# SamsungLabs/SummaryMixing

Hardware: AMD Instinct MI355X
Metric: encoder frames/s (whole node), LibriSpeech Conformer-SummaryMixing (higher is better)
Workload: dtype bf16; 1 GPU; LibriSpeech Conformer-SummaryMixing C2b (12L, d_model=256, d_ffn=1024, SummaryMixing-fast, Swish) training step (fwd+bwd+grad-clip+AdamW); per_gpu_batch=128, enc_frames_per_utt=500, global_batch=128, valid_frames_rank0=49222, input=(B,T,640) N(0,1), wav_len U(0.5,1), zero padded, parallelism=dp1, init=xavier_normal seed 3407, residual_stream=float32 (torch autocast semantics, the reference's `precision: bf16`), launch=eager

## Files before the change

include/smx.h:

```cpp
#ifndef SMX_H_
#define SMX_H_

#include <stddef.h>
#include <stdint.h>

#ifdef __cplusplus
extern "C" {
#endif

#define SMX_VERSION 100

enum { SMX_OK = 0, SMX_EINVAL = -1, SMX_EUNSUPPORTED = -2, SMX_ELAUNCH = -3 };
enum { SMX_F32 = 0, SMX_BF16 = 1 };
enum { SMX_ACT_NONE = 0, SMX_ACT_GELU = 1, SMX_ACT_SWISH = 2, SMX_ACT_LEAKY_RELU = 3, SMX_ACT_RELU = 4 };
enum { SMX_C0_NONE = 0, SMX_C0_ROW = 1, SMX_C0_GROUP = 2, SMX_C0_MOD = 3 };
enum { SMX_GEMM_NT = 0,
       SMX_GEMM_NN = 1,
       SMX_GEMM_TN = 2   };
enum { SMX_OUT_T = 0, SMX_OUT_F32 = 1, SMX_OUT_ATOMIC_F32 = 2 };
enum { SMX_PAD_ZERO = 0, SMX_PAD_REFLECT = 1 };

int smx_version(void);
const char* smx_last_error(void);

// ... 157 lines not shown
  const void* R;       int64_t ldr;
  void* dX;            int64_t lddx;
  float* dgamma;       float* dbeta;
  void* workspace;
  void* dX2;           int64_t lddx2;
  const uint8_t* row_mask2;
  float alpha2;        float drop_p2;
  uint64_t drop_seed2;
  const uint64_t* epoch;
  const void* Z;       int64_t ldz;
  int32_t zact;        int32_t N;
  int32_t D;           int32_t pad_;
} smx_ln_bwd;
int smx_layernorm_bwd(const smx_ln_bwd* a, void* stream);
int smx_layernorm_bwd_blocks(int N);
size_t smx_layernorm_bwd_workspace(int N, int D);

int smx_dwconv1d_glu_fwd(int dtype, const void* P, int64_t ldp, const float* w, const float* bias,
                         const void* gate, int64_t ldg, void* Y, int64_t ldy, int B, int T, int D, int k, int glu,
                         int pad_mode, int chunk, void* stream);
int smx_dwconv1d_glu_fwd_drop(int dtype, const void* P, int64_t ldp, const float* w, const float* bias,
                              const void* gate, int64_t ldg, void* Y, int64_t ldy, int B, int T, int D, int k, int glu,
                              int pad_mode, int chunk, float drop_p, uint64_t drop_seed, const uint64_t* epoch, void* stream);
size_t smx_dwconv1d_glu_bwd_workspace(int B, int T, int D, int k);
int smx_dwconv1d_glu_bwd_partial_rows(int dtype, int B, int T, int D, int k, int glu, int pad_mode, int chunk, int has_gate);
int smx_dwconv1d_glu_bwd(int dtype, const void* dY, int64_t lddy, const void* P, int64_t ldp, const float* w,
                         const float* bias, const void* gate, int64_t ldg, void* dP, int64_t lddp, void* dgate,
                         int64_t lddg, float* dw, float* dbias, int B, int T, int D, int k, int glu, int pad_mode,
                         int chunk, void* workspace, void* stream);

int smx_dft_frames(const float* wav_padded, int64_t ldw, const float* basis_cos, const float* basis_sin, float* spec, int64_t lds,
                   int im_off, int B, int T, int n_fft, int hop, int rows_basis, void* stream);
int smx_frame_window(const float* wav, int64_t ldw, const float* window, float* frames, int B, int L, int T, int n_fft,
                     int hop, void* stream);
size_t smx_fbank_workspace(int B, int T, int n_mels);
int smx_mel_db(int out_dtype, const float* spec, int64_t lds, int im_off, const float* fb, int n_bins, int n_mels,
               float amin, float top_db, void* out, int B, int T, void* workspace, void* stream);
int smx_im2col_s2(int dtype, const void* x, void* col, int B, int T, int F, int C, int Kp, void* stream);
int smx_col2im_s2(int dtype, const void* dcol, void* dx, int B, int T, int F, int C, int Kp, void* stream);
size_t smx_conv1_ln_workspace(int B, int T, int F, int O);
int smx_conv1_ln_fwd(int dtype, const void* X, const float* W9, const float* bias, const float* gamma, const float* beta, float eps,
                     int act, void* Y, float* stats, int B, int T, int F, int O, void* stream);
int smx_conv1_ln_bwd(int dtype, const void* dA, const void* X, const float* W9, const float* bias, const float* gamma,
                     const float* beta, const float* stats, int act, float* grads, void* workspace, int B, int T, int F, int O,
                     void* stream);
int smx_linear_k16_fwd(int dtype, const void* X, const void* W, const float* bias, void* Y, int64_t N, int M, void* stream);
// ... 114 lines not shown
```

summarymixing_amd/_lib.py:

```python
import ctypes
import os

_HERE = os.path.dirname(os.path.abspath(__file__))
LIB_PATH = os.environ.get("SMX_LIB") or os.path.join(_HERE, "libsmx.so")

c_i, c_i64, c_f, c_vp, c_sz = ctypes.c_int, ctypes.c_int64, ctypes.c_float, ctypes.c_void_p, ctypes.c_size_t

F32, BF16 = 0, 1
ACT_NONE, ACT_GELU, ACT_SWISH, ACT_LEAKY_RELU, ACT_RELU = 0, 1, 2, 3, 4
C0_NONE, C0_ROW, C0_GROUP, C0_MOD = 0, 1, 2, 3
GEMM_NT, GEMM_NN, GEMM_TN = 0, 1, 2
OUT_T, OUT_F32, OUT_ATOMIC_F32 = 0, 1, 2
EPI_C0_POST = 1
EPI_ACT_GRAD = 2
EPI_LN_BWD = 4
EPI_LN_FWD = 8
IO_RES_F32, IO_LNX_F32, IO_LNFY_F32 = 1, 2, 4
PAD_ZERO, PAD_REFLECT = 0, 1
ACTS = {"none": ACT_NONE, "identity": ACT_NONE, "gelu": ACT_GELU, "swish": ACT_SWISH,
        "leaky_relu": ACT_LEAKY_RELU, "relu": ACT_RELU}


class ReduceJob(ctypes.Structure):
    _fields_ = [("src", c_vp), ("dst", c_vp), ("src_stride", c_i64), ("ldd", c_i64), ("nsrc", ctypes.c_int32),
# ... 92 lines not shown
    "smx_act_mask_bwd_workspace": (c_sz, [c_i, c_i]),
    "smx_act_mask_bwd": (c_i, [c_i, c_vp, c_i64, c_vp, c_i64, c_vp, c_vp, c_i64, c_i, c_i, c_i, c_f, c_vp, c_vp,
                               c_i64, c_i, c_f, ctypes.c_uint64, c_vp, c_vp, c_vp]),
    "smx_masked_mean_workspace": (c_sz, [c_i, c_i, c_i]),
    "smx_masked_mean_fwd": (c_i, [c_i, c_vp, c_i64, c_vp, c_vp, c_vp, c_i, c_i, c_i, c_i, c_vp, c_vp]),
    "smx_masked_mean_bwd": (c_i, [c_i, c_vp, c_vp, c_vp, c_i64, c_i, c_i, c_i, c_f, ctypes.c_uint64, c_vp, c_vp]),
    "smx_pool_bcast_ok": (c_i, [c_i, c_i, c_i]),
    "smx_pool_bcast": (c_i, [c_i, c_vp, c_i64, c_vp, c_vp, c_vp, c_vp, c_vp, c_i64, c_i, c_i, c_i, c_i, c_f, ctypes.c_uint64, c_vp, c_vp, c_i64,
                             c_vp, c_i, c_vp]),
    "smx_masked_mean_bwd_act": (c_i, [c_i, c_vp, c_vp, c_vp, c_i64, c_vp, c_i64, c_vp, c_i, c_i, c_i, c_i, c_vp]),
    "smx_chunk_mean_workspace": (c_sz, [c_i, c_i, c_i, c_i]),
    "smx_chunk_mean_fwd": (c_i, [c_i, c_vp, c_i64, c_vp, c_i64, c_i, c_i, c_i, c_i, c_i, c_vp, c_vp]),
    "smx_chunk_mean_bwd": (c_i, [c_i, c_vp, c_i64, c_vp, c_i64, c_i, c_i, c_i, c_i, c_i, c_vp, c_vp]),
    "smx_expdecay_mean_workspace": (c_sz, [c_i, c_i, c_i]),
    "smx_expdecay_mean_fwd": (c_i, [c_i, c_vp, c_i64, c_vp, c_i64, c_i, c_i, c_i, c_f, c_vp, c_vp]),
    "smx_expdecay_mean_bwd": (c_i, [c_i, c_vp, c_i64, c_vp, c_i64, c_i, c_i, c_i, c_f, c_vp, c_vp]),
    "smx_layernorm_fwd": (c_i, [ctypes.POINTER(LnFwd), c_vp]),
    "smx_layernorm_bwd_workspace": (c_sz, [c_i, c_i]),
    "smx_layernorm_bwd": (c_i, [ctypes.POINTER(LnBwd), c_vp]),
    "smx_dwconv1d_glu_fwd": (c_i, [c_i, c_vp, c_i64, c_vp, c_vp, c_vp, c_i64, c_vp, c_i64, c_i, c_i, c_i, c_i, c_i,
                                   c_i, c_i, c_vp]),
    "smx_dwconv1d_glu_fwd_drop": (c_i, [c_i, c_vp, c_i64, c_vp, c_vp, c_vp, c_i64, c_vp, c_i64, c_i, c_i, c_i, c_i, c_i,
                                        c_i, c_i, c_f, ctypes.c_uint64, c_vp, c_vp]),
    "smx_dwconv1d_glu_bwd_workspace": (c_sz, [c_i, c_i, c_i, c_i]),
    "smx_dwconv1d_glu_bwd_partial_rows": (c_i, [c_i] * 9),
    "smx_dwconv1d_glu_bwd": (c_i, [c_i, c_vp, c_i64, c_vp, c_i64, c_vp, c_vp, c_vp, c_i64, c_vp, c_i64, c_vp, c_i64,
                                   c_vp, c_vp, c_i, c_i, c_i, c_i, c_i, c_i, c_i, c_vp, c_vp]),
    "smx_dft_frames": (c_i, [c_vp, c_i64, c_vp, c_vp, c_vp, c_i64, c_i, c_i, c_i, c_i, c_i, c_i, c_vp]),
    "smx_frame_window": (c_i, [c_vp, c_i64, c_vp, c_vp, c_i, c_i, c_i, c_i, c_i, c_vp]),
    "smx_fbank_workspace": (c_sz, [c_i, c_i, c_i]),
    "smx_mel_db": (c_i, [c_i, c_vp, c_i64, c_i, c_vp, c_i, c_i, c_f, c_f, c_vp, c_i, c_i, c_vp, c_vp]),
    "smx_im2col_s2": (c_i, [c_i, c_vp, c_vp, c_i, c_i, c_i, c_i, c_i, c_vp]),
    "smx_col2im_s2": (c_i, [c_i, c_vp, c_vp, c_i, c_i, c_i, c_i, c_i, c_vp]),
    "smx_conv1_ln_workspace": (c_sz, [c_i, c_i, c_i, c_i]),
    "smx_conv1_ln_fwd": (c_i, [c_i, c_vp, c_vp, c_vp, c_vp, c_vp, c_f, c_i, c_vp, c_vp, c_i, c_i, c_i, c_i, c_vp]),
    "smx_conv1_ln_bwd": (c_i, [c_i, c_vp, c_vp, c_vp, c_vp, c_vp, c_vp, c_vp, c_i, c_vp, c_vp, c_i, c_i, c_i, c_i, c_vp]),
    "smx_linear_k16_fwd": (c_i, [c_i, c_vp, c_vp, c_vp, c_vp, c_i64, c_i, c_vp]),
    "smx_conv2d_s2_fwd": (c_i, [c_i, c_vp, c_vp, c_vp, c_vp, c_i, c_i, c_i, c_i, c_i, c_i, c_vp]),
    "smx_conv2d_s2_wgrad_workspace": (c_sz, [c_i, c_i, c_i, c_i, c_i]),
    "smx_conv2d_s2_wgrad": (c_i, [c_i, c_vp, c_vp, c_vp, c_vp, c_i, c_i, c_i, c_i, c_i, c_i, c_vp, c_vp]),
    "smx_conv2d_s2_dgrad": (c_i, [c_i, c_vp, c_vp, c_vp, c_i, c_i, c_i, c_i, c_i, c_i, c_vp]),
    "smx_axpby": (c_i, [c_i, c_f, c_vp, c_i64, c_f, c_vp, c_i64, c_vp, c_i64, c_i, c_i, c_vp]),
    "smx_dropout": (c_i, [c_i, c_vp, c_i64, c_vp, c_i64, c_i, c_i, c_f, ctypes.c_uint64, c_vp, c_vp]),
    "smx_add_rowtable": (c_i, [c_i, c_vp, c_i64, c_vp, c_i, c_i, c_i, c_vp]),
    "smx_cast_from_f32": (c_i, [c_i, c_vp, c_vp, c_i64, c_vp]),
    "smx_cast_to_f32": (c_i, [c_i, c_vp, c_vp, c_i64, c_vp]),
# ... 95 lines not shown
```

summarymixing_amd/csrc/dwconv.hip:

```cpp
#include "smx_common.h"

namespace smx {

constexpr int DW_TT = 64;
constexpr int DW_CT = 64;
constexpr int DW_KMAX = 33;
constexpr int DW_ROWS = DW_TT + DW_KMAX - 1;

struct DwParams {
  const void* P; long ldp;
  const float* w; const float* bias;
  const void* gate; long ldg;
  void* Y; long ldy;
  void* dP; long lddp;
  void* dgate; long lddg;
  float* dw; float* dbias;
  int B, T, D, k, glu, pad_mode, chunk;
  unsigned dthresh; float dscale; uint64_t dseed; const uint64_t* epoch;
};

__device__ __forceinline__ int map_frame(int tau, int T, int pad_mode) {
  if (tau >= 0 && tau < T) return tau;
  if (pad_mode == SMX_PAD_REFLECT) {
    int r = tau < 0 ? -tau : 2 * (T - 1) - tau;
    return (r >= 0 && r < T) ? r : -1;
  }
  return -1;
}

template <typename T>
__device__ __forceinline__ void fill_u(float (*u)[DW_CT], const DwParams& p, int b, int t0, int pad, int ch, int cl, int wv) {
  const T* P = reinterpret_cast<const T*>(p.P);
  const int rows = DW_TT + 2 * pad;
  for (int i = wv; i < rows; i += 4) {
    int src = map_frame(t0 - pad + i, p.T, p.pad_mode);
    float val = 0.f;
    if (src >= 0 && ch < p.D) {
      const T* row = P + ((long)b * p.T + src) * p.ldp;
      float a = to_f32(row[ch]);
      val = p.glu ? a * sigmoidf_(to_f32(row[p.D + ch])) : a;
    }
// ... 542 lines not shown
    if (drop_p > 0.f && rk != 2) return fail(SMX_EUNSUPPORTED, "smx_dwconv1d_glu_fwd_drop: fused output dropout needs the rolling CSGU kernel");
    if (rk == 2) {
      p.dthresh = (unsigned)((double)drop_p * 4294967296.0); p.dscale = 1.f / (1.f - drop_p); p.dseed = drop_seed; p.epoch = epoch;
      hipLaunchKernelGGL(dwconv_rollc_fwd, g1, dim3(256), 0, s, p, seg, nseg, gy);
    }
    else if (dtype == SMX_BF16) {
      if (chunk > 0) hipLaunchKernelGGL((dwconv_rolls_fwd<true>), g1, dim3(256), 0, s, p, seg, nseg, gy);
      else hipLaunchKernelGGL((dwconv_rolls_fwd<false>), g1, dim3(256), 0, s, p, seg, nseg, gy);
    } else if (chunk > 0) hipLaunchKernelGGL((dwconv_roll_fwd<float, true>), g1, dim3(256), 0, s, p, seg, nseg, gy);
    else hipLaunchKernelGGL((dwconv_roll_fwd<float, false>), g1, dim3(256), 0, s, p, seg, nseg, gy);
  } else if (drop_p > 0.f) {
    return fail(SMX_EUNSUPPORTED, "smx_dwconv1d_glu_fwd_drop: fused output dropout needs the rolling CSGU kernel");
  } else if (fast) {
    if (gate) {
      if (dtype == SMX_BF16) hipLaunchKernelGGL((dwconv_fwd_fast<bf16_t, 31, true>), grid, dim3(256), 0, s, p);
      else hipLaunchKernelGGL((dwconv_fwd_fast<float, 31, true>), grid, dim3(256), 0, s, p);
    } else {
      if (dtype == SMX_BF16) hipLaunchKernelGGL((dwconv_fwd_fast<bf16_t, 31, false>), grid, dim3(256), 0, s, p);
      else hipLaunchKernelGGL((dwconv_fwd_fast<float, 31, false>), grid, dim3(256), 0, s, p);
    }
  } else if (dtype == SMX_BF16) hipLaunchKernelGGL((dwconv_fwd_kernel<bf16_t>), grid, dim3(256), 0, s, p);
  else hipLaunchKernelGGL((dwconv_fwd_kernel<float>), grid, dim3(256), 0, s, p);
  return check_launch("smx_dwconv1d_glu_fwd");
}

static long tiled_rows(int B, int T, int D) {
  const int tiles_t = (T + DW_TT - 1) / DW_TT, ctiles = (D + DW_CT - 1) / DW_CT;
  long total = (long)B * tiles_t, gy = (1024 + ctiles - 1) / ctiles;
  if (gy > total) gy = total;
  if (gy < 1) gy = 1;
  return gy;
}

extern "C" int smx_dwconv1d_glu_bwd_partial_rows(int dtype, int B, int T, int D, int k, int glu, int pad_mode, int chunk,
                                                 int has_gate) {
  if (B <= 0 || T <= 0 || D <= 0) return 0;
  if (roll_kind(dtype, T, D, k, glu, pad_mode, chunk, has_gate != 0)) {
    int seg, nseg, gy;
    roll_geometry(B, T, D, &seg, &nseg, &gy);
    return gy;
  }
  return (int)tiled_rows(B, T, D);
}

extern "C" size_t smx_dwconv1d_glu_bwd_workspace(int B, int T, int D, int k) {
  if (B <= 0 || T <= 0 || D <= 0) return 0;
// ... 94 lines not shown
```

summarymixing_amd/csrc/dwconv_roll.h:

```cpp
#pragma once

namespace smx {

constexpr int RW_STEP = 16;

template <typename T> struct RwRaw;
template <> struct RwRaw<bf16_t> { typedef unsigned short type; };
template <> struct RwRaw<float> { typedef unsigned int type; };

__device__ __forceinline__ float rw_f32(unsigned short x) { return bf16_bits_to_f32(x); }
__device__ __forceinline__ float rw_f32(unsigned int x) { return __uint_as_float(x); }

template <typename T>
__device__ __forceinline__ typename RwRaw<T>::type rw_ld(__amdgpu_buffer_rsrc_t r, unsigned voff, unsigned soff) {
  if constexpr (sizeof(T) == 2) return __builtin_amdgcn_raw_buffer_load_b16(r, voff, soff, 0);
  else return __builtin_amdgcn_raw_buffer_load_b32(r, voff, soff, 0);
}
template <typename T>
__device__ __forceinline__ void rw_st(float v, __amdgpu_buffer_rsrc_t r, unsigned voff, unsigned soff) {
  if constexpr (sizeof(T) == 2) __builtin_amdgcn_raw_buffer_store_b16((unsigned short)f32_to_bf16_bits(v), r, voff, soff, 0);
  else __builtin_amdgcn_raw_buffer_store_b32(__float_as_uint(v), r, voff, soff, 0);
}

template <typename T>
// ... 243 lines not shown
    out[idx] = ((red[0][a] + red[1][a]) + red[2][a]) + red[3][a];
  }
}

typedef __attribute__((address_space(3))) void* rw_lds_vp;

template <int N> __device__ __forceinline__ void rw_vm() { asm volatile("s_waitcnt vmcnt(%0)" ::"n"(N) : "memory"); }
__device__ __forceinline__ void rw_wait_vm(int n) {
  if (n >= 14) rw_vm<14>(); else if (n >= 10) rw_vm<10>(); else if (n >= 8) rw_vm<8>(); else if (n >= 6) rw_vm<6>();
  else if (n >= 4) rw_vm<4>(); else if (n >= 2) rw_vm<2>(); else rw_vm<0>();
}
__device__ __forceinline__ void rw_lgkm0() { asm volatile("s_waitcnt lgkmcnt(0)" ::: "memory"); }

__device__ __forceinline__ void rw_dma16(__amdgpu_buffer_rsrc_t rs, unsigned char* dst, unsigned vpre, int r0, unsigned ldb) {
  const unsigned s0 = (unsigned)r0 * ldb;
  __builtin_amdgcn_raw_ptr_buffer_load_lds(rs, (rw_lds_vp)dst, 16, vpre + s0, 0, 0, 0);
  __builtin_amdgcn_raw_ptr_buffer_load_lds(rs, (rw_lds_vp)(dst + 1024), 16, vpre + s0 + 8 * ldb, 0, 0, 0);
}

__device__ __forceinline__ float rw_lds_bf16(const unsigned char* base, int off) {
  return bf16_bits_to_f32(*reinterpret_cast<const unsigned short*>(base + off));
}

template <bool CH = false>
__global__ __launch_bounds__(256) void dwconv_rolls_fwd(DwParams p, int seg, int nseg, int gy) {
  constexpr int K = 31, WIN = 46, SLOT = 4096, OUT = 2 * SLOT, WAVE = OUT + 2048;
  __shared__ __attribute__((aligned(16))) unsigned char stage[4][WAVE];
  const int lane = threadIdx.x & 63, wv = __builtin_amdgcn_readfirstlane(threadIdx.x >> 6);
  int iy, bx;
  rw_map(p.D / 64, iy, bx);
  const int item = iy * 4 + wv;
  if (iy >= gy || item >= p.B * nseg) return;
  const int b = item / nseg, t_lo = (item % nseg) * seg, t_hi = min(p.T, t_lo + seg);
  const int nsteps = (t_hi - t_lo + RW_STEP - 1) / RW_STEP;
  const int ch = bx * 64 + lane;
  float w[K];
#pragma unroll
  for (int j = 0; j < K; ++j) w[j] = p.w[(long)ch * K + j];
  const float bs = p.bias ? p.bias[ch] : 0.f;
  bf16_t* Pb = const_cast<bf16_t*>(reinterpret_cast<const bf16_t*>(p.P)) + (long)b * p.T * p.ldp;
  bf16_t* Yb = reinterpret_cast<bf16_t*>(p.Y) + (long)b * p.T * p.ldy;
  const unsigned ldpb = (unsigned)p.ldp * 2, ldyb = (unsigned)p.ldy * 2;
  const __amdgpu_buffer_rsrc_t rP = __builtin_amdgcn_make_buffer_rsrc(Pb, (short)0, (int)(p.T * ldpb), 0x00020000);
  const __amdgpu_buffer_rsrc_t rY = __builtin_amdgcn_make_buffer_rsrc(Yb, (short)0, (int)(p.T * ldyb), 0x00020000);
  const unsigned vcol = (unsigned)(lane & 7) * 16 + (unsigned)bx * 128;
  const unsigned vpa = (unsigned)(lane >> 3) * ldpb + vcol, vpg = vpa + (unsigned)p.D * 2;
  const unsigned vpy = (unsigned)(lane >> 3) * ldyb + vcol;
  unsigned char* st = stage[wv];
  float win[WIN];
#pragma unroll
  for (int i = 0; i < WIN; ++i) win[i] = 0.f;
  auto dma = [&](int s) {
    unsigned char* d = st + (s & 1) * SLOT;
    const int r0 = t_lo + 15 + s * RW_STEP;
    rw_dma16(rP, d, vpa, r0, ldpb);
    rw_dma16(rP, d + 2048, vpg, r0, ldpb);
  };
  const int cz = CH ? p.chunk : 1;
  int m0 = CH ? t_lo % cz : 0;
  dma(-2);
  dma(-1);
  for (int s = -2; s < nsteps; ++s) {
    rw_wait_vm(s < 0 ? 4 : (s >= 2 ? 2 : 0) + (s + 1 < nsteps ? 4 : 0) + (s >= 1 ? 2 : 0));
    const unsigned char* sl = st + (s & 1) * SLOT + lane * 2;
#pragma unroll
    for (int i = 0; i < RW_STEP; ++i) win[30 + i] = rw_lds_bf16(sl, i * 128) * sigmoidf_(rw_lds_bf16(sl, 2048 + i * 128));
    rw_lgkm0();
    if (s + 2 < nsteps) dma(s + 2);
    if (s >= 0) {
      unsigned short* ob = reinterpret_cast<unsigned short*>(st + OUT) + lane;
#pragma unroll
      for (int o = 0; o < RW_STEP; ++o) {
        float acc = bs;
        if constexpr (!CH) {
#pragma unroll
          for (int j = 0; j < K; ++j) acc += w[j] * win[o + j];
        } else {
#pragma unroll
          for (int j = 0; j < 16; ++j) acc += w[j] * win[o + j];
          rw_taps_down(cz - 1 - m0, [&](auto d) { acc += w[15 + decltype(d)::value] * win[o + 15 + decltype(d)::value]; });
          m0 = rw_next(m0, cz);
        }
        ob[o * 64] = (unsigned short)f32_to_bf16_bits(acc);
      }
      asm volatile("" ::: "memory");
      const unsigned s0 = (unsigned)(t_lo + s * RW_STEP) * ldyb;
      typedef uint32_t u32v4 __attribute__((ext_vector_type(4)));
#pragma unroll
      for (int k = 0; k < 2; ++k) {
        const u32v4 v = *reinterpret_cast<const u32v4*>(st + OUT + k * 1024 + lane * 16);
        __builtin_amdgcn_raw_buffer_store_b128(v, rY, vpy + s0 + k * 8 * ldyb, 0, 0);
      }
      asm volatile("" ::: "memory");
    }
#pragma unroll
    for (int i = 0; i < WIN - RW_STEP; ++i) win[i] = win[i + RW_STEP];
  }
}

template <int ABL, bool CH = false>
__global__ __launch_bounds__(256) void dwconv_rolls_bwd(DwParams p, int seg, int nseg, int gy, float* __restrict__ partial) {
  constexpr int K = 31, WIN = 47, SLOT = 6144, OUT = 2 * SLOT, WAVE = OUT + 4096;
  __shared__ float wl[K][64];
  __shared__ __attribute__((aligned(16))) unsigned char stage[4][WAVE];
  const int lane = threadIdx.x & 63, wv = __builtin_amdgcn_readfirstlane(threadIdx.x >> 6);
  int iy, bx;
  rw_map(p.D / 64, iy, bx);
  if (iy >= gy) return;
  const int ch = bx * 64 + lane;
  for (int j = wv; j < K; j += 4) wl[j][lane] = p.w[(long)ch * K + j];
  __syncthreads();
  const int item = iy * 4 + wv;
  float dw[K], dbs = 0.f;
#pragma unroll
  for (int j = 0; j < K; ++j) dw[j] = 0.f;
  if (item < p.B * nseg) {
// ... 388 lines not shown
```

summarymixing_amd/csrc/layernorm.hip:

```cpp
#include <type_traits>

#include "smx_common.h"

namespace smx {

template <typename T, bool VEC>
__global__ __launch_bounds__(256) void layernorm_fwd_kernel(const T* X, long ldx, const float* gamma, const float* beta,
                                                            T* Y, long ldy, float* stats, int N_, int D, float eps,
                                                            int act) {
  const int lane = threadIdx.x & 63;
  const int row = blockIdx.x * 4 + (threadIdx.x >> 6);
  if (row >= N_) return;
  const T* x = X + (long)row * ldx;
  T* y = Y + (long)row * ldy;
  float s = 0.f;
  if (VEC) {
    for (int c = lane * 4; c < D; c += 256) { float f[4]; load4<T>(x + c, f); s += (f[0] + f[1]) + (f[2] + f[3]); }
  } else {
    for (int c = lane; c < D; c += 64) s += to_f32(x[c]);
  }
  const float mean = wave_sum(s) / (float)D;
  float q = 0.f;
  if (VEC) {
    for (int c = lane * 4; c < D; c += 256) {
// ... 187 lines not shown
            if (pass == 0) {
              if (live) {
                typedef uint32_t u32x4n __attribute__((ext_vector_type(4)));
                u32x4n uu = {__float_as_uint(o[0]), __float_as_uint(o[1]), __float_as_uint(o[2]), __float_as_uint(o[3])};
                __builtin_nontemporal_store(uu, reinterpret_cast<u32x4n*>(Y1 + (long)row * ldy1 + c));
              }
#pragma unroll
              for (int j = 0; j < 4; ++j) f[u][i][j] = o[j];
            } else if (live) {
              store4<T2>(Y2 + (long)row * ldy2 + c, o);
            }
          }
        }
      }
    }
  }
}

struct LnSecond {
  void* dX2; long ld; float alpha; const uint8_t* mask; uint32_t thresh; float scale; uint64_t seed; const uint64_t* epoch;
  const float* slabs; int nslab; long slab_stride;
};

template <typename T, int VW, int CH, int U, typename TX = T>
__global__ __launch_bounds__(256) void layernorm_bwd_kernel(const T* __restrict__ dY, long lddy, const TX* __restrict__ X,
                                                            long ldx, const float* __restrict__ gamma,
                                                            const float* __restrict__ beta, int act,
                                                            const float* __restrict__ stats, const T* __restrict__ R,
                                                            long ldr, T* __restrict__ dX, long lddx,
                                                            float* __restrict__ partial, int N_, int D, LnSecond sec) {
  const uint64_t sseed = sec.dX2 ? epoch_seed(sec.seed, sec.epoch) : 0;
  __shared__ float red[3][64];
  const int lane = threadIdx.x & 63, w = threadIdx.x >> 6;
  float gam[CH][VW], bet[CH][VW], dg[CH][VW], db[CH][VW];
#pragma unroll
  for (int i = 0; i < CH; ++i)
#pragma unroll
    for (int j = 0; j < VW; ++j) {
      const int c = (lane + 64 * i) * VW + j;
      gam[i][j] = c < D ? gamma[c] : 0.f;
      bet[i][j] = (c < D && act != SMX_ACT_NONE) ? beta[c] : 0.f;
      dg[i][j] = db[i][j] = 0.f;
    }
  dispatch_act(act, [&](auto act_tag) {
    constexpr int ACT = decltype(act_tag)::value;
    for (int row0 = (blockIdx.x * 4 + w) * U; row0 < N_; row0 += gridDim.x * 4 * U) {
      float fdy[U][CH][VW], fx[U][CH][VW], fr[U][CH][VW == 4 ? 4 : 1], mean[U], rstd[U];
#pragma unroll
      for (int u = 0; u < U; ++u) {
        const int row = min(row0 + u, N_ - 1);
        mean[u] = stats[2 * (long)row];
        rstd[u] = stats[2 * (long)row + 1];
#pragma unroll
        for (int i = 0; i < CH; ++i) {
          const int c = (lane + 64 * i) * VW;
          const int cc = c < D ? c : 0;
          if constexpr (VW == 4) {
            if (sec.slabs) {
              const float* sp = sec.slabs + (long)row * D + cc;
              fdy[u][i][0] = fdy[u][i][1] = fdy[u][i][2] = fdy[u][i][3] = 0.f;
              for (int s0 = 0; s0 < sec.nslab; s0 += 4) {
                float4 a4[4];
#pragma unroll
                for (int k = 0; k < 4; ++k) a4[k] = *reinterpret_cast<const float4*>(sp + (long)min(s0 + k, sec.nslab - 1) * sec.slab_stride);
#pragma unroll
                for (int k = 0; k < 4; ++k)
                  if (s0 + k < sec.nslab) { fdy[u][i][0] += a4[k].x; fdy[u][i][1] += a4[k].y; fdy[u][i][2] += a4[k].z; fdy[u][i][3] += a4[k].w; }
              }
            } else {
              load4<T>(dY + (long)row * lddy + cc, fdy[u][i]);
            }
            load4<TX>(X + (long)row * ldx + cc, fx[u][i]);
          }
          else { fdy[u][i][0] = to_f32(dY[(long)row * lddy + cc]); fx[u][i][0] = to_f32(X[(long)row * ldx + cc]); }
          if constexpr (VW == 4) {
            if (R) load4<T>(R + (long)row * ldr + cc, fr[u][i]);
            else fr[u][i][0] = fr[u][i][1] = fr[u][i][2] = fr[u][i][3] = 0.f;
          }
        }
      }
      float s1[U], s2[U];
// ... 546 lines not shown
                                                           (const TXX*)a.X, a.ldx, a.gamma, a.beta, act, a.stats, (const bf16_t*)a.R, a.ldr, \
                                                           (bf16_t*)a.dX, a.lddx, partial, N, D, (const bf16_t*)ZP, LDZ, ZACT)
  auto ok16 = [](const void* p, int64_t ld) { return rows_ok(p, ld, 16, 8); };
  if (a.Z) {
    if (act != SMX_ACT_NONE)
      return fail(SMX_EUNSUPPORTED, "smx_layernorm_bwd: the pre-activation form is for a LayerNorm without a fused activation of its own");
    if (sizeof(T) != 2 || D > 2048 || D % 8 != 0 || !ok16(a.dY, a.lddy) || !ok16(a.X, a.ldx) || !ok16(a.Z, a.ldz) || !ok16(a.dX, a.lddx))
      return fail(SMX_EUNSUPPORTED, "smx_layernorm_bwd: the pre-activation form needs bf16, D <= 2048, D %% 8 == 0 and 16-byte aligned rows");
    LN_WG8(true, bf16_t, a.Z, a.ldz, a.zact);
    return SMX_OK;
  }
  const size_t vb = 4 * sizeof(T);
  const bool vec = D % 4 == 0 && rows_ok(a.dY, a.lddy, vb, 4) && rows_ok(a.X, a.ldx, 4 * sizeof(TX), 4) && rows_ok(a.R, a.ldr, vb, 4) &&
                   rows_ok(a.dX, a.lddx, vb, 4) && rows_ok(a.dX2, a.lddx2, vb, 4) && (!a.slabs || (aligned16(a.slabs) && a.slab_stride % 4 == 0));
  if (a.dX2 && D > 2048) return fail(SMX_EUNSUPPORTED, "smx_layernorm_bwd: the second output needs D <= 2048");
  if ((x32 || a.slabs) && !(vec && D <= 2048))
    return fail(SMX_EUNSUPPORTED, "smx_layernorm_bwd: float32 X and slabs need D %% 4 == 0, D <= 2048 and aligned rows");
  if (sizeof(T) == 2 && vec && !a.slabs && !a.dX2 && D > SMX_LN_WG8_FROM && D <= 2048 && D % 8 == 0 && ok16(a.dY, a.lddy) && ok16(a.X, a.ldx) &&
      ok16(a.R, a.ldr) && ok16(a.dX, a.lddx)) {
    LN_WG8(false, TX, nullptr, 0, SMX_ACT_NONE);
    return SMX_OK;
  }
#undef LN_WG8
#define LN_ROWS(VW, CH, U) hipLaunchKernelGGL((layernorm_bwd_kernel<T, VW, CH, U, TX>), grid, dim3(256), 0, s, (const T*)a.dY, a.lddy, (const TX*)a.X, a.ldx, \
                                              a.gamma, a.beta, act, a.stats, (const T*)a.R, a.ldr, (T*)a.dX, a.lddx, partial, N, D, sec)
#define LN_WIDE(KERNEL, CH) hipLaunchKernelGGL((KERNEL<T, CH>), grid, dim3(256), 0, s, (const T*)a.dY, a.lddy, (const T*)a.X, a.ldx, a.gamma, a.beta, \
                                               act, a.stats, (const T*)a.R, a.ldr, (T*)a.dX, a.lddx, partial, N, D)
  if (vec && D <= 2048) {
    if (!a.slabs) {
      if (D <= 256) LN_ROWS(4, 1, SMX_LNB_U1); else if (D <= 512) LN_ROWS(4, 2, SMX_LNB_U2); else if (D <= 1024) LN_ROWS(4, 4, 1); else LN_ROWS(4, 8, 1);
    } else if constexpr (sizeof(T) == 2) {
      if (D <= 256) LN_ROWS(4, 1, 1); else if (D <= 512) LN_ROWS(4, 2, 1); else if (D <= 1024) LN_ROWS(4, 4, 1); else LN_ROWS(4, 8, 1);
    }
  } else if constexpr (std::is_same<T, TX>::value) {
    if (vec) {
      if (D <= 3072) LN_WIDE(layernorm_bwd_wide4_kernel, 3);
      else if (D <= 4096) LN_WIDE(layernorm_bwd_wide4_kernel, 4);
      else return fail(SMX_EUNSUPPORTED, "smx_layernorm_bwd: D=%d > 4096", D);
    } else {
      if (D <= 256) LN_ROWS(1, 4, 1); else if (D <= 1024) LN_ROWS(1, 16, 1); else if (D <= 2048) LN_ROWS(1, 32, 1);
      else if (D <= 4096) LN_WIDE(layernorm_bwd_wide_kernel, 16);
      else return fail(SMX_EUNSUPPORTED, "smx_layernorm_bwd: D=%d > 4096", D);
    }
  }
#undef LN_WIDE
#undef LN_ROWS
  return SMX_OK;
}

extern "C" int smx_layernorm_bwd(const smx_ln_bwd* a, void* stream) {
  SMX_REQUIRE(a && a->X && a->gamma && a->beta && a->stats && a->dX && a->workspace && a->D > 0 && ((a->dgamma == nullptr) == (a->dbeta == nullptr)),
              "smx_layernorm_bwd: bad arguments");
  SMX_REQUIRE((a->dY == nullptr) != (a->slabs == nullptr), "smx_layernorm_bwd: exactly one of dY and slabs");
  SMX_REQUIRE(!a->slabs || (a->dtype == SMX_BF16 && a->nslab >= 1 && a->nslab <= 16 && !a->dgamma),
              "smx_layernorm_bwd: slabs need bf16, 1 <= nslab <= 16 and dgamma = dbeta = NULL");
// ... 19 lines not shown
```

summarymixing_amd/functional.py:

```python
import weakref

import collections
import ctypes
import os

import torch

from . import _lib as L
from . import ops
from . import sequence_parallel as SP

_PANEL = os.environ.get("SMX_PANEL", "1") != "0"
_PANEL_MIN_ROWS = int(os.environ.get("SMX_PANEL_MIN_ROWS", "2048"))

_SPLITK = os.environ.get("SMX_SPLITK", "1") != "0"
_SPLITK_MAX_ROWS = int(os.environ.get("SMX_SPLITK_MAX_ROWS", "2048"))

_LN_FUSE, _LN_FUSE_FWD, _LN_FUSE_BWD = (os.environ.get("SMX_LN_FUSE", "1").lower() != off for off in ("0", "bwd", "fwd"))
_LN_FUSE_MIN_ROWS = int(os.environ.get("SMX_LN_FUSE_MIN_ROWS", "17500"))
_LN_PAIR = True

_POOL_FUSE = os.environ.get("SMX_POOL_FUSE", "1") != "0"

RESIDUAL_F32 = os.environ.get("SMX_RESIDUAL", "fp32").lower() not in ("bf16", "bfloat16")

_DEFER_REDUCE = os.environ.get("SMX_DEFER_REDUCE", "1") != "0"
_WGRAD_GROUP = os.environ.get("SMX_WGRAD_GROUP", "1") != "0"
_WGRAD_DIRECT_MAX_ROWS = int(os.environ.get("SMX_WGRAD_DIRECT_MAX_ROWS", "8192"))

_shadow = {}


def register_shadow(param, shadow):
    _shadow[id(param)] = (weakref.ref(param), "managed", None, shadow)
    for key in [k for k in _packed if k[0] == id(param)]:
        del _packed[key]
    weights_changed()


def wcast(param, dtype):
    if dtype == torch.float32:
        return param.detach()
    ent = _shadow.get(id(param))
# ... 969 lines not shown

    def bwd(dy, dz_in=None, second=None):
        if dz_in is not None:
            dz1, _ = linear_bwd(dz_in, a, W2, None, L.ACT_NONE, None, 1.0, gacc(P["W2"]), gacc(P["b2"]), dz_ready=True,
                                up=(z1, act, None, 1.0, d1, None), wparam=P["W2"])
        else:
            dz1, _ = linear_bwd(dy, a, W2, None, L.ACT_NONE, None, alpha, gacc(P["W2"]), gacc(P["b2"]), drop=d2,
                                up=(z1, act, None, 1.0, d1, None), wparam=P["W2"])
        return dgrad_ln_bwd(ln_b, dz1, h, W1, P["W1"], P["b1"], z1, act, res=dy, second=second, dz_ready=True)
    bwd.pre = (alpha, None, d2)
    return ret(bwd)

def conv_module_fwd(x, P, act, mask, B, T, need_bwd, dtype, chunk=0, residual=True, p=0.0, pre_ln=None, ln_next=None,
                    conv_state=None, conv_slots=None):
    d = x.shape[1]
    if SP.enabled():
        r = _conv_module_fwd_sp(x, P, act, mask, B, T, need_bwd, dtype, chunk, residual, p)
        return r + (None,) if ln_next is not None else r
    h, ln1_b = ln_fwd(x, P["ln1_w"], P["ln1_b"], 1e-5, need_bwd, pre=pre_ln, out_dtype=dtype)
    Wp = wcast(P["Wp"], dtype).view(2 * d, d)
    p_, _ = linear_fwd(h, Wp, P["bp"], wparam=P["Wp"])
    k = P["wd"].shape[-1]
    wd = P["wd"].detach().reshape(d, k)
    if conv_state is None:
        c = ops.dwconv_fwd(p_, wd, P["bd"].detach() if P["bd"] is not None else None, B, T, d, k, True, L.PAD_ZERO, chunk)
    else:
        if need_bwd:
            raise NotImplementedError("streaming convolution: inference only")
        if conv_slots is None:
            c = ops.dwconv_stream(p_, wd, P["bd"].detach() if P["bd"] is not None else None, conv_state, B, T, d, k)
        else:
            c = ops.dwconv_slots(p_, wd, P["bd"].detach() if P["bd"] is not None else None, conv_state, *conv_slots, B, T, d, k)
    a, ln2_b = ln_fwd(c, P["ln2_w"], P["ln2_b"], 1e-5, need_bwd, act)
    Wo = wcast(P["Wo"], dtype)
    dr = (p, ops.new_dropout_seed()) if p > 0.0 else None
    post = []
    lnn = None if ln_next is None else LnNext(ln_next[0], ln_next[1], ln_next[2], need_bwd)
    y, _ = linear_fwd(a, Wo, P["bo"], L.ACT_NONE, mask, res=x if residual else None, drop=dr, ln_next=lnn, ln_post=post, wparam=P["Wo"])
    post = post[0] if post else None
    if not need_bwd:
        return (y, None, post) if ln_next is not None else (y, None)

    def bwd(dy, dz_in=None, second=None):
        dc = (dgrad_ln_bwd(ln2_b, dz_in, a, Wo, P["Wo"], P["bo"], packed=False, dz_ready=True) if dz_in is not None else
              dgrad_ln_bwd(ln2_b, dy, a, Wo, P["Wo"], P["bo"], mask=mask, packed=False, drop=dr))
        gwd = gacc(P["wd"])
        dp, _ = dwconv_bwd_deferred(dc, p_, wd, P["bd"].detach() if P["bd"] is not None else None, gwd.view(d, k),
                                    gacc(P["bd"]), B, T, d, k, True, L.PAD_ZERO, chunk)
        return dgrad_ln_bwd(ln1_b, dp, h, Wp, P["Wp"], P["bp"], res=dy if residual else None, second=second)
    bwd.pre = (1.0, mask, dr) if (mask is not None or dr is not None) else None
    bwd.ln1_fused = ln_fusable(ln1_b.spec, h.shape[0], d, dtype, 2 * d, Wp)
    return (y, bwd, post) if ln_next is not None else (y, bwd)


def _conv_module_fwd_sp(x, P, act, mask, B, T, need_bwd, dtype, chunk, residual, p):
    d = x.shape[1]
# ... 132 lines not shown
```

summarymixing_amd/ops.py:

```python
import ctypes


import torch

from . import _lib as L

_DT = {torch.float32: L.F32, torch.bfloat16: L.BF16}


def dt(t):
    try:
        return _DT[t.dtype]
    except KeyError:
        raise TypeError(f"summarymixing_amd supports float32 and bfloat16 activations, got {t.dtype}")


def _stream():
    return ctypes.c_void_p(torch.cuda.current_stream().cuda_stream)


def _p(t):
    return ctypes.c_void_p(t.data_ptr()) if t is not None else None


# ... 528 lines not shown

def layernorm_bwd_preact(dy, x, gamma, beta, stats, z, zact, dgamma, dbeta, act=L.ACT_NONE, ws=None, dx_out=None):
    return layernorm_bwd(dy, x, gamma, beta, stats, dgamma, dbeta, act=act, ws=ws, dx_out=dx_out, preact=(z, zact))


def dwconv_fwd(p, w, bias, B, T, D, k, glu, pad_mode=L.PAD_ZERO, chunk=0, gate=None, drop=None):
    y = torch.empty((B * T, D), dtype=p.dtype, device=p.device)
    pp, ldp = _mat(p)
    pg, ldg = (_mat(gate) if gate is not None else (None, 0))
    tok = _pb(f"dwconv_fwd ({B},{T},{D}) k={k}", 3 * B * T * D * _es(p))
    fused = False
    if drop is not None and drop[0] > 0.0 and _CSGU_DROP_FUSE:
        fused = L.lib().smx_dwconv1d_glu_fwd_drop(dt(p), pp, ldp, _p(w), _p(bias), pg, ldg, _p(y), D, B, T, D, k, 1 if glu else 0,
                                                  pad_mode, chunk, drop[0], drop[1], _epoch(), _stream()) == 0
    if not fused:
        L.check(L.lib().smx_dwconv1d_glu_fwd(dt(p), pp, ldp, _p(w), _p(bias), pg, ldg, _p(y), D, B, T, D, k, 1 if glu else 0,
                                             pad_mode, chunk, _stream()), "smx_dwconv1d_glu_fwd")
    _pe(tok)
    if drop is not None and drop[0] > 0.0 and not fused:
        dropout(y, drop[0], drop[1], out=y)
    return y


def dwconv_stream(p, w, bias, state, B, C_cur, D, k):
    assert state.dtype == p.dtype and state.is_contiguous() and state.shape == (B, (k - 1) // 2, 2 * D)
    y = torch.empty((B * C_cur, D), dtype=p.dtype, device=p.device)
    pp, ldp = _mat(p)
    tok = _pb(f"dwconv_stream ({B},{C_cur},{D}) k={k}", 3 * B * C_cur * D * _es(p))
    L.check(L.lib().smx_dwconv1d_glu_stream(dt(p), pp, ldp, _p(w), _p(bias), _p(state), _p(y), D, B, C_cur, D, k, _stream()),
            "smx_dwconv1d_glu_stream")
    _pe(tok)
    return y


def stream_advance(counter, table, pe, C):
    assert table.dtype == pe.dtype
    pt, ldt = _mat(table)
    pp, ldpe = _mat(pe)
    L.check(L.lib().smx_stream_advance(dt(pe), _p(counter), pt, ldt, table.shape[0], pp, ldpe, C, pe.shape[1], _stream()),
            "smx_stream_advance")


def slot_summary(s, out, B, C, left, ring, counters, valid):
    D = s.shape[1]
    ps, lds = _mat(s)
    po, ldo = _mat(out)
# ... 539 lines not shown
```

Before: 3.616 million encoder frames/s.

## Fuse LayerNorm and activation into the rolling depthwise-conv GLU forward kernel

Adds a variant of the rolling depthwise-conv kernel that also computes the following LayerNorm (mean/rstd via cross-wave LDS reduction in double) and the Swish/GELU activation. It writes the conv output, the normalized activated output and the row stats in one pass. This removes a separate LayerNorm forward launch and its re-read of the conv output in the conv module. The work split changes from one wave per channel tile to four waves covering all 256 channels of a time segment, with extra barriers per step. Separately, the slab branch in the LayerNorm backward becomes a compile-time template flag.

```diff
diff --git a/include/smx.h b/include/smx.h
--- a/include/smx.h
+++ b/include/smx.h
@@ -203,6 +203,10 @@
 int smx_dwconv1d_glu_fwd_drop(int dtype, const void* P, int64_t ldp, const float* w, const float* bias,
                               const void* gate, int64_t ldg, void* Y, int64_t ldy, int B, int T, int D, int k, int glu,
                               int pad_mode, int chunk, float drop_p, uint64_t drop_seed, const uint64_t* epoch, void* stream);
+int smx_dwconv1d_glu_ln_ok(int dtype, int T, int D, int k, int glu, int pad_mode, int chunk, int act);
+int smx_dwconv1d_glu_ln_fwd(int dtype, const void* P, int64_t ldp, const float* w, const float* bias, void* Y, int64_t ldy,
+                            const float* gamma, const float* beta, float eps, int act, void* A, int64_t lda, float* stats,
+                            int B, int T, int D, int k, void* stream);
 size_t smx_dwconv1d_glu_bwd_workspace(int B, int T, int D, int k);
 int smx_dwconv1d_glu_bwd_partial_rows(int dtype, int B, int T, int D, int k, int glu, int pad_mode, int chunk, int has_gate);
 int smx_dwconv1d_glu_bwd(int dtype, const void* dY, int64_t lddy, const void* P, int64_t ldp, const float* w,
diff --git a/summarymixing_amd/_lib.py b/summarymixing_amd/_lib.py
--- a/summarymixing_amd/_lib.py
+++ b/summarymixing_amd/_lib.py
@@ -138,6 +138,9 @@
                                    c_i, c_i, c_vp]),
     "smx_dwconv1d_glu_fwd_drop": (c_i, [c_i, c_vp, c_i64, c_vp, c_vp, c_vp, c_i64, c_vp, c_i64, c_i, c_i, c_i, c_i, c_i,
                                         c_i, c_i, c_f, ctypes.c_uint64, c_vp, c_vp]),
+    "smx_dwconv1d_glu_ln_ok": (c_i, [c_i] * 8),
+    "smx_dwconv1d_glu_ln_fwd": (c_i, [c_i, c_vp, c_i64, c_vp, c_vp, c_vp, c_i64, c_vp, c_vp, c_f, c_i, c_vp, c_i64, c_vp, c_i, c_i, c_i,
+                                      c_i, c_vp]),
     "smx_dwconv1d_glu_bwd_workspace": (c_sz, [c_i, c_i, c_i, c_i]),
     "smx_dwconv1d_glu_bwd_partial_rows": (c_i, [c_i] * 9),
     "smx_dwconv1d_glu_bwd": (c_i, [c_i, c_vp, c_i64, c_vp, c_i64, c_vp, c_vp, c_vp, c_i64, c_vp, c_i64, c_vp, c_i64,
diff --git a/summarymixing_amd/csrc/dwconv.hip b/summarymixing_amd/csrc/dwconv.hip
--- a/summarymixing_amd/csrc/dwconv.hip
+++ b/summarymixing_amd/csrc/dwconv.hip
@@ -17,6 +17,7 @@
   float* dw; float* dbias;
   int B, T, D, k, glu, pad_mode, chunk;
   unsigned dthresh; float dscale; uint64_t dseed; const uint64_t* epoch;
+  const float* ln_gamma; const float* ln_beta; float ln_eps; void* A; long lda; float* ln_stats;
 };
 
 __device__ __forceinline__ int map_frame(int tau, int T, int pad_mode) {
@@ -605,6 +606,37 @@
   } else if (dtype == SMX_BF16) hipLaunchKernelGGL((dwconv_fwd_kernel<bf16_t>), grid, dim3(256), 0, s, p);
   else hipLaunchKernelGGL((dwconv_fwd_kernel<float>), grid, dim3(256), 0, s, p);
   return check_launch("smx_dwconv1d_glu_fwd");
+}
+
+extern "C" int smx_dwconv1d_glu_ln_ok(int dtype, int T, int D, int k, int glu, int pad_mode, int chunk, int act) {
+  return dtype == SMX_BF16 && D == 256 && T > 0 && chunk <= 0 && (act == SMX_ACT_SWISH || act == SMX_ACT_GELU) &&
+         roll_kind(dtype, T, D, k, glu, pad_mode, chunk, false) == 1;
+}
+
+extern "C" int smx_dwconv1d_glu_ln_fwd(int dtype, const void* P, int64_t ldp, const float* w, const float* bias, void* Y, int64_t ldy,
+                                       const float* gamma, const float* beta, float eps, int act, void* A, int64_t lda, float* stats,
+                                       int B, int T, int D, int k, void* stream) {
+  SMX_REQUIRE(P && w && Y && gamma && beta && A && stats, "smx_dwconv1d_glu_ln_fwd: null pointer");
+  if (B <= 0 || T <= 0) return SMX_OK;
+  if (!smx_dwconv1d_glu_ln_ok(dtype, T, D, k, 1, SMX_PAD_ZERO, 0, act))
+    return fail(SMX_EUNSUPPORTED, "smx_dwconv1d_glu_ln_fwd: bf16, D = 256, k = 31, Swish or GELU only (smx_dwconv1d_glu_ln_ok)");
+  if (!(ldp % 8 == 0 && ldy % 8 == 0 && lda % 8 == 0 && ldp >= 2 * D && ldy >= D && lda >= D && aligned16(P) && aligned16(Y) && aligned16(A) &&
+        reinterpret_cast<uintptr_t>(stats) % 8 == 0))
+    return fail(SMX_EUNSUPPORTED, "smx_dwconv1d_glu_ln_fwd: rows and bases must be 16-byte aligned");
+  const long ldmax = ldp > ldy ? (ldp > lda ? ldp : lda) : (ldy > lda ? ldy : lda);
+  SMX_REQUIRE((long)T * ldmax * 4 < (1L << 31), "smx_dwconv1d_glu_ln_fwd: utterance span >= 2 GB");
+  DwParams p;
+  memset(&p, 0, sizeof(p));
+  p.P = P; p.ldp = ldp; p.w = w; p.bias = bias; p.Y = Y; p.ldy = ldy;
+  p.B = B; p.T = T; p.D = D; p.k = k; p.glu = 1; p.pad_mode = SMX_PAD_ZERO;
+  p.ln_gamma = gamma; p.ln_beta = beta; p.ln_eps = eps; p.A = A; p.lda = lda; p.ln_stats = stats;
+  int seg, nseg, gy;
+  roll_geometry(B, T, D, &seg, &nseg, &gy);
+  const dim3 g1((unsigned)(8 * 4 * ((gy + 7) / 8)));
+  hipStream_t s = reinterpret_cast<hipStream_t>(stream);
+  if (act == SMX_ACT_SWISH) hipLaunchKernelGGL((dwconv_rolls_fwd<false, SMX_ACT_SWISH>), g1, dim3(256), 0, s, p, seg, nseg, gy);
+  else hipLaunchKernelGGL((dwconv_rolls_fwd<false, SMX_ACT_GELU>), g1, dim3(256), 0, s, p, seg, nseg, gy);
+  return check_launch("smx_dwconv1d_glu_ln_fwd");
 }
 
 static long tiled_rows(int B, int T, int D) {
diff --git a/summarymixing_amd/csrc/dwconv_roll.h b/summarymixing_amd/csrc/dwconv_roll.h
--- a/summarymixing_amd/csrc/dwconv_roll.h
+++ b/summarymixing_amd/csrc/dwconv_roll.h
@@ -289,18 +289,22 @@
   return bf16_bits_to_f32(*reinterpret_cast<const unsigned short*>(base + off));
 }
 
-template <bool CH = false>
+template <bool CH = false, int LNACT = -1>
 __global__ __launch_bounds__(256) void dwconv_rolls_fwd(DwParams p, int seg, int nseg, int gy) {
   constexpr int K = 31, WIN = 46, SLOT = 4096, OUT = 2 * SLOT, WAVE = OUT + 2048;
+  constexpr bool LN = LNACT >= 0;
+  constexpr int NST = LN ? 5 : 2;
+  static_assert(!(CH && LN), "the fused LayerNorm is not part of the Dynamic Chunk Convolution kernel");
   __shared__ __attribute__((aligned(16))) unsigned char stage[4][WAVE];
   const int lane = threadIdx.x & 63, wv = __builtin_amdgcn_readfirstlane(threadIdx.x >> 6);
   int iy, bx;
-  rw_map(p.D / 64, iy, bx);
-  const int item = iy * 4 + wv;
+  rw_map(LN ? 4 : p.D / 64, iy, bx);
+  const int item = iy * 4 + (LN ? bx : wv);
+  const int ct = LN ? wv : bx;
   if (iy >= gy || item >= p.B * nseg) return;
   const int b = item / nseg, t_lo = (item % nseg) * seg, t_hi = min(p.T, t_lo + seg);
   const int nsteps = (t_hi - t_lo + RW_STEP - 1) / RW_STEP;
-  const int ch = bx * 64 + lane;
+  const int ch = ct * 64 + lane;
   float w[K];
 #pragma unroll
   for (int j = 0; j < K; ++j) w[j] = p.w[(long)ch * K + j];
@@ -310,9 +314,19 @@
   const unsigned ldpb = (unsigned)p.ldp * 2, ldyb = (unsigned)p.ldy * 2;
   const __amdgpu_buffer_rsrc_t rP = __builtin_amdgcn_make_buffer_rsrc(Pb, (short)0, (int)(p.T * ldpb), 0x00020000);
   const __amdgpu_buffer_rsrc_t rY = __builtin_amdgcn_make_buffer_rsrc(Yb, (short)0, (int)(p.T * ldyb), 0x00020000);
-  const unsigned vcol = (unsigned)(lane & 7) * 16 + (unsigned)bx * 128;
+  const unsigned vcol = (unsigned)(lane & 7) * 16 + (unsigned)ct * 128;
   const unsigned vpa = (unsigned)(lane >> 3) * ldpb + vcol, vpg = vpa + (unsigned)p.D * 2;
   const unsigned vpy = (unsigned)(lane >> 3) * ldyb + vcol;
+  const unsigned ldab = LN ? (unsigned)p.lda * 2 : 0u;
+  const unsigned vpo = (unsigned)(lane >> 3) * ldab + vcol;
+  __amdgpu_buffer_rsrc_t rA = rY, rS = rY;
+  float lng = 0.f, lnb = 0.f;
+  if constexpr (LN) {
+    rA = __builtin_amdgcn_make_buffer_rsrc(reinterpret_cast<bf16_t*>(p.A) + (long)b * p.T * p.lda, (short)0, (int)(p.T * ldab), 0x00020000);
+    rS = __builtin_amdgcn_make_buffer_rsrc(p.ln_stats + 2 * (long)b * p.T, (short)0, p.T * 8, 0x00020000);
+    lng = p.ln_gamma[ch]; lnb = p.ln_beta[ch];
+    asm volatile("" :: "v"(lng), "v"(lnb));
+  }
   unsigned char* st = stage[wv];
   float win[WIN];
 #pragma unroll
@@ -328,7 +342,7 @@
   dma(-2);
   dma(-1);
   for (int s = -2; s < nsteps; ++s) {
-    rw_wait_vm(s < 0 ? 4 : (s >= 2 ? 2 : 0) + (s + 1 < nsteps ? 4 : 0) + (s >= 1 ? 2 : 0));
+    rw_wait_vm(s < 0 ? 4 : (s >= 2 ? NST : 0) + (s + 1 < nsteps ? 4 : 0) + (s >= 1 ? NST : 0));
     const unsigned char* sl = st + (s & 1) * SLOT + lane * 2;
 #pragma unroll
     for (int i = 0; i < RW_STEP; ++i) win[30 + i] = rw_lds_bf16(sl, i * 128) * sigmoidf_(rw_lds_bf16(sl, 2048 + i * 128));
@@ -359,6 +373,81 @@
         __builtin_amdgcn_raw_buffer_store_b128(v, rY, vpy + s0 + k * 8 * ldyb, 0, 0);
       }
       asm volatile("" ::: "memory");
+      if constexpr (LN) {
+        const int f = lane >> 2, q = lane & 3;
+        float cf[16], cown[RW_STEP];
+        {
+          const u32v4 u0 = *reinterpret_cast<const u32v4*>(st + OUT + f * 128 + q * 32);
+          const u32v4 u1 = *reinterpret_cast<const u32v4*>(st + OUT + f * 128 + q * 32 + 16);
+          const uint32_t uw[8] = {u0.x, u0.y, u0.z, u0.w, u1.x, u1.y, u1.z, u1.w};
+#pragma unroll
+          for (int i = 0; i < 8; ++i) { cf[2 * i] = __uint_as_float(uw[i] << 16); cf[2 * i + 1] = __uint_as_float(uw[i] & 0xffff0000u); }
+        }
+#pragma unroll
+        for (int o = 0; o < RW_STEP; ++o) cown[o] = bf16_bits_to_f32(ob[o * 64]);
+        double sm = 0.0, sq = 0.0;
+#pragma unroll
+        for (int i = 0; i < 16; ++i) { const double x = (double)cf[i]; sm += x; sq = __builtin_fma(x, x, sq); }
+        sm += __shfl_xor(sm, 1, 64); sq += __shfl_xor(sq, 1, 64);
+        sm += __shfl_xor(sm, 2, 64); sq += __shfl_xor(sq, 2, 64);
+        rw_lgkm0();
+        asm volatile("" ::: "memory");
+        if (q == 0) {
+          const uint64_t u0 = (uint64_t)__double_as_longlong(sm), u1 = (uint64_t)__double_as_longlong(sq);
+          const u32v4 pk = {(uint32_t)u0, (uint32_t)(u0 >> 32), (uint32_t)u1, (uint32_t)(u1 >> 32)};
+          asm volatile("ds_write_b128 %0, %1" ::"v"((unsigned)(uintptr_t)(rw_lds_vp)(st + OUT + f * 16)), "v"(pk) : "memory");
+        }
+        rw_lgkm0();
+        __builtin_amdgcn_s_barrier();
+        asm volatile("" ::: "memory");
+        float mean, rstd;
+        {
+          const int ff = lane & 15;
+          u32v4 pr[4];
+          asm volatile("ds_read_b128 %0, %4\n\tds_read_b128 %1, %4 offset:%5\n\tds_read_b128 %2, %4 offset:%6\n\tds_read_b128 %3, %4 offset:%7\n\t"
+                       "s_waitcnt lgkmcnt(0)"
+                       : "=&v"(pr[0]), "=&v"(pr[1]), "=&v"(pr[2]), "=&v"(pr[3])
+                       : "v"((unsigned)(uintptr_t)(rw_lds_vp)(&stage[0][OUT + ff * 16])), "n"(WAVE), "n"(2 * WAVE), "n"(3 * WAVE)
+                       : "memory");
+          double ts = 0.0, tq = 0.0;
+#pragma unroll
+          for (int k = 0; k < 4; ++k) {
+            ts += __longlong_as_double((long long)((uint64_t)pr[k].x | ((uint64_t)pr[k].y << 32)));
+            tq += __longlong_as_double((long long)((uint64_t)pr[k].z | ((uint64_t)pr[k].w << 32)));
+          }
+          const double mu = ts * (1.0 / 256.0);
+          const double var = fmax(tq * (1.0 / 256.0) - mu * mu, 0.0);
+          mean = (float)mu;
+          const double ve = var + (double)p.ln_eps;
+          double y = (double)rsqrtf((float)ve);
+#pragma unroll
+          for (int it = 0; it < 2; ++it) y = __builtin_fma(0.5 * y, __builtin_fma(-ve * y, y, 1.0), y);
+          rstd = (float)y;
+        }
+        rw_lgkm0();
+        __builtin_amdgcn_s_barrier();
+        asm volatile("" ::: "memory");
+        {
+          typedef uint32_t u32v2 __attribute__((ext_vector_type(2)));
+          const u32v2 sv = {__float_as_uint(mean), __float_as_uint(rstd)};
+          const unsigned so = (lane < 16 && (lane >> 2) == wv) ? (unsigned)(t_lo + s * RW_STEP + lane) * 8u : 0x80000000u;
+          __builtin_amdgcn_raw_buffer_store_b64(sv, rS, so, 0, 0);
+        }
+#pragma unroll
+        for (int o = 0; o < RW_STEP; ++o) {
+          const float mo = __builtin_bit_cast(float, __builtin_amdgcn_readlane(__builtin_bit_cast(int, mean), o));
+          const float ro = __builtin_bit_cast(float, __builtin_amdgcn_readlane(__builtin_bit_cast(int, rstd), o));
+          ob[o * 64] = (unsigned short)f32_to_bf16_bits(act_fwd_c<LNACT>((cown[o] - mo) * ro * lng + lnb));
+        }
+        asm volatile("" ::: "memory");
+        const unsigned a0 = (unsigned)(t_lo + s * RW_STEP) * ldab;
+#pragma unroll
+        for (int k = 0; k < 2; ++k) {
+          const u32v4 v = *reinterpret_cast<const u32v4*>(st + OUT + k * 1024 + lane * 16);
+          __builtin_amdgcn_raw_buffer_store_b128(v, rA, vpo + a0 + k * 8 * ldab, 0, 0);
+        }
+        asm volatile("" ::: "memory");
+      }
     }
 #pragma unroll
     for (int i = 0; i < WIN - RW_STEP; ++i) win[i] = win[i + RW_STEP];
diff --git a/summarymixing_amd/csrc/layernorm.hip b/summarymixing_amd/csrc/layernorm.hip
--- a/summarymixing_amd/csrc/layernorm.hip
+++ b/summarymixing_amd/csrc/layernorm.hip
@@ -233,7 +233,7 @@
   const float* slabs; int nslab; long slab_stride;
 };
 
-template <typename T, int VW, int CH, int U, typename TX = T>
+template <typename T, int VW, int CH, int U, typename TX = T, bool SLAB = false>
 __global__ __launch_bounds__(256) void layernorm_bwd_kernel(const T* __restrict__ dY, long lddy, const TX* __restrict__ X,
                                                             long ldx, const float* __restrict__ gamma,
                                                             const float* __restrict__ beta, int act,
@@ -267,7 +267,7 @@
           const int c = (lane + 64 * i) * VW;
           const int cc = c < D ? c : 0;
           if constexpr (VW == 4) {
-            if (sec.slabs) {
+            if constexpr (SLAB) {
               const float* sp = sec.slabs + (long)row * D + cc;
               fdy[u][i][0] = fdy[u][i][1] = fdy[u][i][2] = fdy[u][i][3] = 0.f;
               for (int s0 = 0; s0 < sec.nslab; s0 += 4) {
@@ -860,7 +860,7 @@
     return SMX_OK;
   }
 #undef LN_WG8
-#define LN_ROWS(VW, CH, U) hipLaunchKernelGGL((layernorm_bwd_kernel<T, VW, CH, U, TX>), grid, dim3(256), 0, s, (const T*)a.dY, a.lddy, (const TX*)a.X, a.ldx, \
+#define LN_ROWS(VW, CH, U, ...) hipLaunchKernelGGL((layernorm_bwd_kernel<T, VW, CH, U, TX, ##__VA_ARGS__>), grid, dim3(256), 0, s, (const T*)a.dY, a.lddy, (const TX*)a.X, a.ldx, \
                                               a.gamma, a.beta, act, a.stats, (const T*)a.R, a.ldr, (T*)a.dX, a.lddx, partial, N, D, sec)
 #define LN_WIDE(KERNEL, CH) hipLaunchKernelGGL((KERNEL<T, CH>), grid, dim3(256), 0, s, (const T*)a.dY, a.lddy, (const T*)a.X, a.ldx, a.gamma, a.beta, \
                                                act, a.stats, (const T*)a.R, a.ldr, (T*)a.dX, a.lddx, partial, N, D)
@@ -868,7 +868,7 @@
     if (!a.slabs) {
       if (D <= 256) LN_ROWS(4, 1, SMX_LNB_U1); else if (D <= 512) LN_ROWS(4, 2, SMX_LNB_U2); else if (D <= 1024) LN_ROWS(4, 4, 1); else LN_ROWS(4, 8, 1);
     } else if constexpr (sizeof(T) == 2) {
-      if (D <= 256) LN_ROWS(4, 1, 1); else if (D <= 512) LN_ROWS(4, 2, 1); else if (D <= 1024) LN_ROWS(4, 4, 1); else LN_ROWS(4, 8, 1);
+      if (D <= 256) LN_ROWS(4, 1, 1, true); else if (D <= 512) LN_ROWS(4, 2, 1, true); else if (D <= 1024) LN_ROWS(4, 4, 1, true); else LN_ROWS(4, 8, 1, true);
     }
   } else if constexpr (std::is_same<T, TX>::value) {
     if (vec) {
diff --git a/summarymixing_amd/functional.py b/summarymixing_amd/functional.py
--- a/summarymixing_amd/functional.py
+++ b/summarymixing_amd/functional.py
@@ -19,6 +19,7 @@
 _LN_FUSE, _LN_FUSE_FWD, _LN_FUSE_BWD = (os.environ.get("SMX_LN_FUSE", "1").lower() != off for off in ("0", "bwd", "fwd"))
 _LN_FUSE_MIN_ROWS = int(os.environ.get("SMX_LN_FUSE_MIN_ROWS", "17500"))
 _LN_PAIR = True
+_DWCONV_LN = os.environ.get("SMX_DWCONV_LN", "1") != "0"
 
 _POOL_FUSE = os.environ.get("SMX_POOL_FUSE", "1") != "0"
 
@@ -1034,7 +1035,12 @@
     p_, _ = linear_fwd(h, Wp, P["bp"], wparam=P["Wp"])
     k = P["wd"].shape[-1]
     wd = P["wd"].detach().reshape(d, k)
-    if conv_state is None:
+    ln2_pre = None
+    if conv_state is None and _DWCONV_LN and ops.dwconv_ln_ok(p_, B, T, d, k, act, chunk):
+        c, a_, st_ = ops.dwconv_ln_fwd(p_, wd, P["bd"].detach() if P["bd"] is not None else None, P["ln2_w"].detach(), P["ln2_b"].detach(),
+                                       1e-5, act, B, T, d, k)
+        ln2_pre = (a_, st_)
+    elif conv_state is None:
         c = ops.dwconv_fwd(p_, wd, P["bd"].detach() if P["bd"] is not None else None, B, T, d, k, True, L.PAD_ZERO, chunk)
     else:
         if need_bwd:
@@ -1043,7 +1049,7 @@
             c = ops.dwconv_stream(p_, wd, P["bd"].detach() if P["bd"] is not None else None, conv_state, B, T, d, k)
         else:
             c = ops.dwconv_slots(p_, wd, P["bd"].detach() if P["bd"] is not None else None, conv_state, *conv_slots, B, T, d, k)
-    a, ln2_b = ln_fwd(c, P["ln2_w"], P["ln2_b"], 1e-5, need_bwd, act)
+    a, ln2_b = ln_fwd(c, P["ln2_w"], P["ln2_b"], 1e-5, need_bwd, act, pre=ln2_pre)
     Wo = wcast(P["Wo"], dtype)
     dr = (p, ops.new_dropout_seed()) if p > 0.0 else None
     post = []
diff --git a/summarymixing_amd/ops.py b/summarymixing_amd/ops.py
--- a/summarymixing_amd/ops.py
+++ b/summarymixing_amd/ops.py
@@ -574,6 +574,23 @@
     return y
 
 
+def dwconv_ln_ok(p, B, T, D, k, act, chunk=0):
+    return (p.dtype == torch.bfloat16 and p.stride(1) == 1 and p.stride(0) % 8 == 0 and p.data_ptr() % 16 == 0
+            and L.lib().smx_dwconv1d_glu_ln_ok(dt(p), T, D, k, 1, L.PAD_ZERO, chunk, act) == 1)
+
+
+def dwconv_ln_fwd(p, w, bias, gamma, beta, eps, act, B, T, D, k):
+    c = torch.empty((B * T, D), dtype=p.dtype, device=p.device)
+    a = torch.empty((B * T, D), dtype=p.dtype, device=p.device)
+    stats = torch.empty((B * T, 2), dtype=torch.float32, device=p.device)
+    pp, ldp = _mat(p)
+    tok = _pb(f"dwconv_ln_fwd ({B},{T},{D}) k={k}", 4 * B * T * D * _es(p))
+    L.check(L.lib().smx_dwconv1d_glu_ln_fwd(dt(p), pp, ldp, _p(w), _p(bias), _p(c), D, _p(gamma), _p(beta), eps, act, _p(a), D, _p(stats),
+                                            B, T, D, k, _stream()), "smx_dwconv1d_glu_ln_fwd")
+    _pe(tok)
+    return c, a, stats
+
+
 def dwconv_stream(p, w, bias, state, B, C_cur, D, k):
     assert state.dtype == p.dtype and state.is_contiguous() and state.shape == (B, (k - 1) // 2, 2 * D)
     y = torch.empty((B * C_cur, D), dtype=p.dtype, device=p.device)
```

Result: no change. 3.641 million encoder frames/s, median of 6 (+0.7%).
